# hadleyhzy34/porl

Measured on AMD Instinct MI355X. Metric: gradient-steps/sec (POR update, batch=1024), higher is better.
Workload: dtype f32; 1 GPU; POR S=60 A=2 H=1024 L=2 B=1024/GPU (global 1024), 1000000 -row replay (1000000/GPU) resident in HBM, device sampler + gather + full update per step; parallelism=dp1, global_batch=1024

## Files before the change

### include/porl_hip.h

```cpp
#ifndef PORL_HIP_H
#define PORL_HIP_H

#include <stdint.h>

#ifdef __cplusplus
extern "C" {
#endif

#define PORL_ABI_VERSION 11
#define PORL_MAX_HIDDEN 8

#define PORL_OK 0
#define PORL_ERR_INVALID (-1)
#define PORL_ERR_UNSUPPORTED (-2)
#define PORL_ERR_UNBOUND (-3)

int porl_abi_version(void);
const char* porl_last_error(void);

typedef struct porl_iql_cfg {
  int32_t obs_dim;
  int32_t pol_out_dim;
  int32_t hidden_dim;
  int32_t n_hidden;
  int32_t layer_norm;
  int32_t pol_tanh;
  int32_t weight_mode;
  int32_t max_batch;
} porl_iql_cfg;

typedef struct porl_iql porl_iql;

int porl_iql_create(const porl_iql_cfg* cfg, porl_iql** out);
void porl_iql_destroy(porl_iql* h);

int64_t porl_iql_group_floats(const porl_iql* h, int group);
int32_t porl_iql_group_tensors(const porl_iql* h, int group);
int porl_iql_tensor_info(const porl_iql* h, int group, int index, int64_t* offset, int32_t* rows,
                         int32_t* cols);

int64_t porl_iql_workspace_floats(const porl_iql* h);

typedef struct porl_iql_buffers {
  float* params_vf;
  float* params_tgt;
  float* params_pol;
  float* grads_vf;
  float* grads_pol;
  float* adam_m_vf;
  float* adam_v_vf;
  float* adam_m_pol;
  float* adam_v_pol;
  float* workspace;
  float* stats;
} porl_iql_buffers;

int porl_iql_bind(porl_iql* h, const porl_iql_buffers* bufs);

int porl_iql_load_batch(porl_iql* h, int32_t batch,
                        const float* obs, int64_t obs_rs,
                        const float* next_obs, int64_t next_rs,
                        const float* rew, int64_t rew_rs,
                        const float* term, int64_t term_rs,
                        const float* pol_target, int64_t pt_rs,
// ... 428 lines not shown
```

### porl_amd/_native.py

```python
from __future__ import annotations

import ctypes as C
import os

_HERE = os.path.dirname(os.path.abspath(__file__))
LIB_PATH = os.path.join(_HERE, "lib", "libporl_hip.so")

ABI_VERSION = 11

SYMBOLS = [
    "porl_abi_version", "porl_last_error",
    "porl_iql_create", "porl_iql_destroy", "porl_iql_group_floats", "porl_iql_group_tensors",
    "porl_iql_tensor_info", "porl_iql_workspace_floats", "porl_iql_bind", "porl_iql_load_batch",
    "porl_iql_load_batch_sampled", "porl_iql_load_batch_indexed", "porl_iql_set_stats", "porl_iql_set_mode", "porl_iql_tune_set",
    "porl_iql_value_backward", "porl_iql_value_apply", "porl_iql_policy_forward", "porl_iql_policy_backward",
    "porl_iql_policy_apply", "porl_iql_step", "porl_iql_policy_only_forward", "porl_iql_policy_only_step", "porl_iql_policy_prefetch", "porl_iql_forward_value", "porl_iql_forward_policy",
    "porl_gemm_f32", "porl_gemm_f32_group", "porl_adam_ema", "porl_ema", "porl_softmax_mask", "porl_gather_rows", "porl_sample_indices", "porl_epoch_indices", "porl_per_update", "porl_per_sample",
    "porl_per_record", "porl_per_sample_slots", "porl_per_update_f32",
    "porl_prof_enable", "porl_prof_read", "porl_tune_set", "porl_tune_set_ptr", "porl_state2costmap", "porl_astar_label",
    "porl_signal_create", "porl_signal_destroy", "porl_signal_write", "porl_signal_wait_ge", "porl_iql_update_pipelined",
    "porl_qnet_create", "porl_qnet_destroy", "porl_qnet_param_floats", "porl_qnet_tensors",
    "porl_qnet_tensor_info", "porl_qnet_workspace_floats", "porl_qnet_bind", "porl_qnet_load_batch",
    "porl_qnet_cql_backward", "porl_qnet_apply", "porl_qnet_learn", "porl_qnet_sync_target",
    "porl_qnet_forward", "porl_qnet_forward_loaded", "porl_qnet_backward", "porl_qr_loss", "porl_iqn_quantile_huber", "porl_iqn_cos_embed", "porl_iqn_hadamard", "porl_iqn_hadamard_backward", "porl_iqn_select", "porl_iqn_scatter", "porl_iqn_target", "porl_grad_clip", "porl_c51_loss", "porl_reduce_mean", "porl_qnet_penalty", "porl_qnet_learn_indexed", "porl_qnet_one_launch", "porl_qnet_learn_variant", "porl_qnet_can_sample", "porl_qnet_learn_sampled", "porl_qnet_dist_learn",
    "porl_qnet_record", "porl_qnet_act_ok", "porl_qnet_act",
    "porl_qnet_learn_sampled_variant", "porl_qnet_bcq_mask", "porl_qnet_bcq_learn", "porl_qnet_bcq_learn_sampled",
    "porl_iqn_create", "porl_iqn_destroy", "porl_iqn_workspace_floats", "porl_iqn_bind", "porl_iqn_learn", "porl_iqn_act",
    "porl_iqn_mix", "porl_iqn_head",
    "porl_enc_create", "porl_enc_destroy", "porl_enc_param_floats", "porl_enc_stat_floats",
    "porl_enc_workspace_floats", "porl_enc_tensors", "porl_enc_norms", "porl_enc_blocks",
    "porl_enc_tensor_info", "porl_enc_norm_info", "porl_enc_bind", "porl_enc_weights_changed", "porl_enc_forward", "porl_enc_forward_rows",
    "porl_enc_tap_info",
    "porl_episode_workspace", "porl_episode_count", "porl_episode_fill", "porl_episode_returns", "porl_hindsight_pairs",
    "porl_gather_pairs",
]

# ... 97 lines not shown


class NativeError(RuntimeError):
    pass


_lib = None


def _declare(lib):
    vp, i32, i64, f32, f64 = C.c_void_p, C.c_int32, C.c_int64, C.c_float, C.c_double
    lib.porl_abi_version.restype = C.c_int
    lib.porl_last_error.restype = C.c_char_p
    lib.porl_iql_create.argtypes = [C.POINTER(IqlCfg), C.POINTER(vp)]
    lib.porl_iql_destroy.argtypes = [vp]
    lib.porl_iql_destroy.restype = None
    lib.porl_iql_group_floats.argtypes = [vp, C.c_int]
    lib.porl_iql_group_floats.restype = i64
    lib.porl_iql_group_tensors.argtypes = [vp, C.c_int]
    lib.porl_iql_group_tensors.restype = i32
    lib.porl_iql_tensor_info.argtypes = [vp, C.c_int, C.c_int, C.POINTER(i64), C.POINTER(i32), C.POINTER(i32)]
    lib.porl_iql_workspace_floats.argtypes = [vp]
    lib.porl_iql_workspace_floats.restype = i64
    lib.porl_iql_bind.argtypes = [vp, C.POINTER(IqlBuffers)]
    lib.porl_iql_load_batch.argtypes = [vp, i32, vp, i64, vp, i64, vp, i64, vp, i64, vp, i64, vp]
    lib.porl_iql_load_batch_sampled.argtypes = [vp, i32, vp, i64, i64, i32, i32, C.c_uint64, C.c_uint64, vp, vp]
    lib.porl_iql_load_batch_indexed.argtypes = [vp, i32, vp, i64, i64, vp, i32, i32, i32, i32, vp, i64, vp, i64, vp]
    lib.porl_iql_set_stats.argtypes = [vp, vp]
    lib.porl_iql_set_mode.argtypes = [vp, i32]
    for name in ("porl_iql_value_backward", "porl_iql_value_apply", "porl_iql_policy_forward", "porl_iql_policy_backward",
                 "porl_iql_policy_apply", "porl_iql_step", "porl_iql_policy_only_forward", "porl_iql_policy_only_step"):
        getattr(lib, name).argtypes = [vp, C.POINTER(IqlHyper), vp]
    lib.porl_iql_policy_prefetch.argtypes = [vp, vp]
    lib.porl_iql_forward_value.argtypes = [vp, C.c_int, vp, i64, i32, vp, vp, vp]
    lib.porl_iql_forward_policy.argtypes = [vp, vp, i64, i32, vp, i64, vp]
    lib.porl_gemm_f32.argtypes = [C.c_int, C.c_int, i32, i32, i32, vp, i32, vp, i32, vp, i32, vp, C.c_int,
                                  vp, i32, C.c_int, vp, vp]
    lib.porl_gemm_f32_group.argtypes = [C.POINTER(GemmDesc), i32, C.c_int, C.c_int, vp]
    lib.porl_adam_ema.argtypes = [vp, vp, vp, vp, vp, i64, f64, i32, f64, f64, f64, f64, vp]
    lib.porl_ema.argtypes = [vp, vp, i64, f64, vp]
    lib.porl_softmax_mask.argtypes = [vp, i64, i32, i32, f32, i32, vp, vp]
    lib.porl_gather_rows.argtypes = [vp, i64, vp, i32, i32, vp, i64, vp]
    lib.porl_sample_indices.argtypes = [i64, i32, C.c_uint64, C.c_uint64, i64, vp, vp]
    lib.porl_epoch_indices.argtypes = [i64, i64, i32, C.c_uint64, C.c_uint64, i64, vp, vp]
    lib.porl_per_update.argtypes = [vp, i64, vp, vp, i32, f64, f64, vp, vp]
    lib.porl_per_sample.argtypes = [vp, i64, vp, i32, i64, f64, vp, vp, vp, vp]
# ... 141 lines not shown
```

### porl_amd/csrc/gemm_f32.hpp

```cpp
#pragma once
#include <hip/hip_runtime.h>
#include <stdint.h>

#ifndef PORL_ABL
#define PORL_ABL 0
#endif

namespace porl {

enum : int { ACT_NONE = 0, ACT_RELU = 1, ACT_TANH = 2 };

enum : int {
  APRO_NONE = 0,
  APRO_AFFINE_RELU = 1,
};

struct GemmProb {
  const float* A;
  const float* B;
  float* C;
  const float* bias;
  const float* mask;
  const float* headw;
  float* headout;
  float* colsum;
  const float* a_colscale;
  const float* a_colshift;
  const float* resid;
  const float* rscale;
  float* cstat;
  int rs_rows, rs_row0;
  int a_grp, a_grp_jump, a_seg_tiles, a_seg_jump;
  int M, N, K;
  int lda, ldb, ldc, ldmask;
  int act;
  int apro;
  int splitk;
  int store_c;
  int a_vec, b_vec;
  int a_kc, b_kc;
  int c_vec;
  int tiles_m, tiles_n, block_start, kchunk;
};

constexpr int MAX_GROUP = 8;
struct GemmGroup {
  int nprob;
  int total_blocks;
  int single_buffer;
  GemmProb p[MAX_GROUP];
  int lds_pad, lds_pad_min_blocks;
};

// ... 20 lines not shown
  const unsigned long long a = reinterpret_cast<unsigned long long>(p);
  BufRsrc r;
  r.x = (int)(unsigned)(a & 0xFFFFFFFFull);
  r.y = (int)(unsigned)((a >> 32) & 0xFFFFull);
  r.z = (int)(bytes >= 0x7FFFFFFFull ? 0x7FFFFFFFu : (unsigned)bytes);
  r.w = 0x00020000;
  return r;
}
__device__ __forceinline__ float4 buf_ld128(BufRsrc r, unsigned voff, unsigned soff) {
  const f32x4 v = llvm_raw_buffer_load_v4f32(r, (int)voff, (int)soff, 0);
  return make_float4(v.x, v.y, v.z, v.w);
}
__device__ __forceinline__ float buf_ld32(BufRsrc r, unsigned voff, unsigned soff) {
  return llvm_raw_buffer_load_f32(r, (int)voff, (int)soff, 0);
}

template <bool V> struct BoolTag { static constexpr bool value = V; };
template <int V> struct IntTag { static constexpr int value = V; };

#ifdef PORL_STAMP
__device__ unsigned long long g_stamps[16 * 4096];
#endif

template <int BM, int BN, int BK, int WM, int WN, bool VEC, bool APRO, bool ONEBUF = false>
__global__ __launch_bounds__(64 * WM * WN) void gemm_f32_kernel(const GemmGroup g) {
  constexpr int THREADS = 64 * WM * WN;
  constexpr int WTM = BM / WM / 32;
  constexpr int WTN = BN / WN / 32;
  constexpr int SA = lds_stride(BM);
  constexpr int SB = lds_stride(BN);
  constexpr int SK = BK + 4;
  constexpr int A_TILE = (BK * SA > BM * SK) ? BK * SA : BM * SK;
  constexpr int B_TILE = (BK * SB > BN * SK) ? BK * SB : BN * SK;
  static_assert(BK % 8 == 0, "a k-group is 8 wide");
  constexpr int NLA = BM * BK / 4 / THREADS;
  constexpr int NLB = BN * BK / 4 / THREADS;
  static_assert(NLA >= 1 && NLB >= 1, "tile too small for the thread count");
  static_assert(BM * BK / 4 % THREADS == 0 && BN * BK / 4 % THREADS == 0, "staging must divide evenly");
  static_assert(BK % 4 == 0 && WTM >= 1 && WTN >= 1 && BM % (32 * WM) == 0 && BN % (32 * WN) == 0, "tile shape");

  constexpr int APRO_MAX_K = ONEBUF ? 512 : 1024;
  constexpr int NBUF = ONEBUF ? 1 : 2;
  __shared__ __attribute__((aligned(16))) float lds[NBUF * (A_TILE + B_TILE) + (APRO ? 2 * APRO_MAX_K : 0)];

  const int t = threadIdx.x;
  const int lane = t & 63;
  const int wave = t >> 6;
// ... 379 lines not shown

  auto run = [&](auto guard_tag) {
    if (a_kc && b_kc) {
      main_loop(guard_tag, BoolTag<true>{}, BoolTag<true>{}, BoolTag<false>{});
    } else if constexpr (APRO) {
    } else if (a_kc) {
      main_loop(guard_tag, BoolTag<true>{}, BoolTag<false>{}, BoolTag<false>{});
    } else if (do_colsum) {
      main_loop(guard_tag, BoolTag<false>{}, BoolTag<false>{}, BoolTag<true>{});
    } else {
      main_loop(guard_tag, BoolTag<false>{}, BoolTag<false>{}, BoolTag<false>{});
    }
  };
  if constexpr (VEC) {
    if (full) run(BoolTag<false>{});
    else run(BoolTag<true>{});
  } else {
    run(BoolTag<true>{});
  }
#ifdef PORL_STAMP
  if (t == 0) { rt_loop1 = __builtin_amdgcn_s_memrealtime(); cy1 = __builtin_amdgcn_s_memtime(); }
#endif

  if (do_colsum) {
    __syncthreads();
    float4* red = reinterpret_cast<float4*>(lds);
    constexpr int C4 = BM / 4;
    auto reduce_cols = [&](const float4& mine, float* out) {
      red[t] = mine;
      __syncthreads();
      if (t < C4) {
        float4 s = red[t];
        for (int u = t + C4; u < THREADS; u += C4) {
          const float4 o = red[u];
          s.x += o.x; s.y += o.y; s.z += o.z; s.w += o.w;
        }
        const int c = m0 + t * 4;
        if (c < M) out[c] = s.x;
        if (c + 1 < M) out[c + 1] = s.y;
        if (c + 2 < M) out[c + 2] = s.z;
        if (c + 3 < M) out[c + 3] = s.w;
      }
      __syncthreads();
    };
    reduce_cols(csum, P.colsum + (size_t)split * M);
  }

  const bool raw = P.splitk > 1;
  float* __restrict__ Cg = P.C + (raw ? (size_t)split * M * P.ldc : 0);
  const bool has_head = (!raw) && P.headw != nullptr;
  const float* __restrict__ maskp = raw ? nullptr : P.mask;
  const int act = raw ? ACT_NONE : P.act;
  const bool store_c = P.store_c != 0;
  constexpr int WROWS = BM / WM, WCOLS = BN / WN, CS = WCOLS + 4;
  static_assert(WM * WN * WROWS * CS <= NBUF * (A_TILE + B_TILE), "C sub-tiles must fit in the staging LDS");
  const bool fast_c = store_c && P.c_vec && (m0 + BM <= M) && (n0 + BN <= N);
  float* ctile = lds + wave * (WROWS * CS);
#pragma unroll
  for (int i = 0; i < WTM; ++i) {
    const int rbase = m0 + wm * (BM / WM) + i * 32 + 4 * kh;
#pragma unroll
    for (int j = 0; j < WTN; ++j) {
      const int col = n0 + wn * (BN / WN) + j * 32 + li;
      const bool col_ok = col < N;
      float bv = 0.f, hw = 0.f;
      if (!raw && col_ok) {
        if (P.bias) bv = P.bias[col];
        if (has_head) hw = P.headw[col];
      }
      float vals[16];
#pragma unroll
      for (int r = 0; r < 16; ++r) {
        float v = acc[i][j][r] + bv;
        if (act == ACT_RELU) v = fmaxf(v, 0.f);
        else if (act == ACT_TANH) v = tanhf(v);
        vals[r] = v;
      }
      if (maskp && !fast_c) {
#pragma unroll
        for (int r = 0; r < 16; ++r) {
// ... 25 lines not shown
        cs += __shfl_xor(cs, 32);
        cq += __shfl_xor(cq, 32);
        const int rblk = (m0 + wm * (BM / WM)) / 32 + i;
        if (kh == 0 && col_ok && rblk * 32 < M) {
          float* o = P.cstat + (size_t)rblk * 2 * N + col;
          o[0] = cs;
          o[N] = cq;
        }
      }
      if (has_head) {
        const int part = (n0 + wn * (BN / WN) + j * 32) >> 5;
#pragma unroll
        for (int r = 0; r < 16; ++r) {
          float sh = vals[r] * hw;
          sh += __shfl_xor(sh, 16);
          sh += __shfl_xor(sh, 8);
          sh += __shfl_xor(sh, 4);
          sh += __shfl_xor(sh, 2);
          sh += __shfl_xor(sh, 1);
          const int row = rbase + (r & 3) + 8 * (r >> 2);
          if (li == 0 && row < M && part * 32 < N) P.headout[(size_t)part * M + row] = sh;
        }
      }
      if (store_c) {
        if (fast_c) {
#pragma unroll
          for (int r = 0; r < 16; ++r)
            ctile[(i * 32 + (r & 3) + 8 * (r >> 2) + 4 * kh) * CS + j * 32 + li] = vals[r];
        } else {
#pragma unroll
          for (int r = 0; r < 16; ++r) {
            const int row = rbase + (r & 3) + 8 * (r >> 2);
            if (row < M && col_ok) Cg[(size_t)row * P.ldc + col] = vals[r];
          }
        }
      }
    }
  }
  if (fast_c) {
    constexpr int C4 = WCOLS / 4;
    const int wr0 = m0 + wm * WROWS, wc0 = n0 + wn * WCOLS;
#pragma unroll 4
    for (int f = lane; f < WROWS * C4; f += 64) {
      const int r = f / C4, c = (f % C4) * 4;
      float4 v = *reinterpret_cast<const float4*>(ctile + r * CS + c);
      if (maskp) {
        const float4 mk = *reinterpret_cast<const float4*>(maskp + (size_t)(wr0 + r) * P.ldmask + wc0 + c);
        v.x = mk.x > 0.f ? v.x : 0.f; v.y = mk.y > 0.f ? v.y : 0.f;
        v.z = mk.z > 0.f ? v.z : 0.f; v.w = mk.w > 0.f ? v.w : 0.f;
      }
      if (!raw && P.resid) {
        const float rs = P.rscale ? P.rscale[(wr0 + r + P.rs_row0) / P.rs_rows] : 1.f;
        const float4 x4 = *reinterpret_cast<const float4*>(P.resid + (size_t)(wr0 + r) * P.ldc + wc0 + c);
        v.x = __fadd_rn(x4.x, __fmul_rn(v.x, rs)); v.y = __fadd_rn(x4.y, __fmul_rn(v.y, rs));
        v.z = __fadd_rn(x4.z, __fmul_rn(v.z, rs)); v.w = __fadd_rn(x4.w, __fmul_rn(v.w, rs));
      }
      *reinterpret_cast<float4*>(Cg + (size_t)(wr0 + r) * P.ldc + wc0 + c) = v;
    }
// ... 65 lines not shown
    if (p.splitk < 1) p.splitk = 1;
    int kc = (p.K + p.splitk - 1) / p.splitk;
    kc = ((kc + GEMM_BK - 1) / GEMM_BK) * GEMM_BK;
    p.kchunk = kc;
    p.c_vec = aligned16(p.C) && (p.ldc % 4 == 0) && (p.splitk == 1 || ((size_t)p.M * p.ldc) % 4 == 0) &&
              (p.mask == nullptr || (aligned16(p.mask) && p.ldmask % 4 == 0));
    p.block_start = start;
    start += p.tiles_m * p.tiles_n * p.splitk;
  }
  g.total_blocks = start;
  return start;
}

template <int BM, int BN, int WM, int WN>
inline hipError_t launch_tile(const GemmGroup& g, hipStream_t s) {
  dim3 grid(g.total_blocks), block(64 * WM * WN);
  const int pad = g.total_blocks >= g.lds_pad_min_blocks ? g.lds_pad : 0;
  bool vec = true, apro = g.p[0].apro != APRO_NONE;
  for (int i = 0; i < g.nprob; ++i) {
    vec = vec && g.p[i].a_vec && g.p[i].b_vec;
    if ((g.p[i].apro != APRO_NONE) != apro) return hipErrorInvalidValue;
    if (g.p[i].splitk <= 1 && (g.p[i].mask || g.p[i].resid) && (g.p[i].cstat || g.p[i].headw)) return hipErrorInvalidValue;
  }
  if (apro) {
    if constexpr ((BM == 64 && BN == 64) || (BM == 128 && BN == 64) || (BM == 128 && BN == 96)) {
      for (int i = 0; i < g.nprob; ++i) {
        const GemmProb& p = g.p[i];
        if (!p.a_kc || !p.b_kc || p.K % GEMM_BK || p.splitk > 1 || !p.a_colscale || !p.a_colshift || !vec ||
            (reinterpret_cast<uintptr_t>(p.a_colscale) & 15u) || (reinterpret_cast<uintptr_t>(p.a_colshift) & 15u))
          return hipErrorInvalidValue;
        if (p.K > (g.single_buffer && BM == 64 && BN == 64 ? 512 : 1024)) return hipErrorInvalidValue;
      }
      if constexpr (BM == 64 && BN == 64) {
        if (g.single_buffer) {
          hipLaunchKernelGGL((gemm_f32_kernel<BM, BN, GEMM_BK, WM, WN, true, true, true>), grid, block, pad, s, g);
          return hipGetLastError();
        }
      }
      hipLaunchKernelGGL((gemm_f32_kernel<BM, BN, GEMM_BK, WM, WN, true, true>), grid, block, pad, s, g);
      return hipGetLastError();
    } else {
      return hipErrorInvalidValue;
    }
  }
  if constexpr (BM == 64 && BN == 64) {
    if (vec && g.single_buffer) {
// ... 38 lines not shown
```

### porl_amd/csrc/porl_api.hip

```cpp
#include <hip/hip_runtime.h>

#include <algorithm>
#include <cmath>
#include <cstdio>
#include <cstring>
#include <string>
#include <vector>

#include "../../include/porl_hip.h"
#include "gemm_f32.hpp"
#include "gemm_bf16.hpp"
#include "kernels.hpp"
#include "l0_fwd.hpp"
#include "skinny.hpp"
#include "iqn.hpp"
#include "qnet_fused.hpp"
#include "per_tree.hpp"
#include "dist_losses.hpp"
#include "online.hpp"
#include "per_online.hpp"
#include "bcq_mask.hpp"
#include "astar.hpp"
#include "episodes.hpp"

// ... 85 lines not shown
    (void)hipEventRecord(r.e1, s);
    g_prof.recs.push_back(r);
  }
};

const float* g_dbg_a_scale = nullptr; const float* g_dbg_a_shift = nullptr; const float* g_dbg_resid = nullptr;
float* g_dbg_cstat = nullptr;
unsigned long long* g_qnet_stamps = nullptr;

constexpr int NUM_CU = 256;
constexpr int SK_MAX = 16;
constexpr int NLL_ROWS_PER_BLOCK = 4;
constexpr int LN_ROWS_PER_BLOCK = 8;
constexpr int HEAD_ROWS_PER_BLOCK = HEAD_ROWS;

struct Tune {
  int tile_map[4] = {TILE_64x128, TILE_64x64, TILE_64x128, TILE_64x64};
  int tile_map_short[4] = {TILE_64x64, TILE_64x64, TILE_64x128, TILE_64x64};
  int vbwd_tile_short = -1;
  int l0_kernel = 1;
  int l0_tile = -1;
  int skinny = 7;
  int skinny_pipelined = -1, skinny_pipelined_max_h = 768;
  int dw0_slabs = 16;
  int iql_fold = 1;
  int gemm_lds_pad = 0, gemm_lds_pad_min_blocks = 0;
  int iql_pad_value = 18432, iql_pad_policy = 0, iql_pad_min_blocks = 4 * NUM_CU, iql_pad_min_k = 0;
  int enc_tile_n96 = 0;
  int enc_gemm_sb = 1;
  int enc_patch_rows = 0;
  int enc_s2d = 0;
  int enc_bf16_operands_only = 0;
  int enc_pconv_mfma = 0;
  int enc_bn_sweep = 0;
  int enc_dense_patch = 0;
  int qnet_fused = 1;
  int qnet_rows16 = 1;
  int qnet_wgrad_share = 11;
  int qnet_two_groups = 1;
} g_tune;

enum TuneClamp { TC_ANY, TC_BOOL, TC_NONNEG, TC_1_16, TC_MASK };
struct TuneKey { const char* key; int Tune::*field; TuneClamp clamp; };
#define TK(key, clamp) {#key, &Tune::key, clamp}
const TuneKey k_tune_keys[] = {
    TK(gemm_lds_pad, TC_NONNEG), TK(gemm_lds_pad_min_blocks, TC_NONNEG), TK(iql_pad_value, TC_NONNEG), TK(iql_pad_policy, TC_NONNEG),
    TK(iql_pad_min_blocks, TC_NONNEG), TK(iql_pad_min_k, TC_NONNEG), TK(qnet_fused, TC_BOOL), TK(qnet_two_groups, TC_BOOL),
    TK(qnet_wgrad_share, TC_1_16), TK(qnet_rows16, TC_BOOL), TK(enc_dense_patch, TC_BOOL), TK(enc_s2d, TC_BOOL), TK(enc_patch_rows, TC_NONNEG),
    TK(enc_gemm_sb, TC_ANY), TK(enc_tile_n96, TC_BOOL), TK(enc_bn_sweep, TC_BOOL), TK(enc_pconv_mfma, TC_BOOL), TK(enc_bf16_operands_only, TC_BOOL),
    TK(iql_fold, TC_BOOL), TK(skinny, TC_MASK), TK(skinny_pipelined, TC_MASK), TK(skinny_pipelined_max_h, TC_ANY), TK(dw0_slabs, TC_1_16),
    TK(l0_tile, TC_ANY), TK(l0_kernel, TC_BOOL), TK(vbwd_tile_short, TC_ANY),
};

int tune_apply(Tune& t, const char* key, int value) {
  if (!key) PORL_FAIL(PORL_ERR_INVALID, "null key");
  for (const TuneKey& k : k_tune_keys) {
    if (strcmp(key, k.key)) continue;
    const TuneClamp c = k.clamp;
    t.*k.field = c == TC_BOOL ? value != 0 : c == TC_NONNEG ? std::max(0, value) : c == TC_1_16 ? std::max(1, std::min(value, 16))
               : c == TC_MASK && value == 1 ? 7 : value;
    return PORL_OK;
  }
  const bool sh = !strncmp(key, "tile_map_short", 14);
  const char* i = key + (sh ? 14 : 8);
  if (!strncmp(key, "tile_map", 8) && *i >= '0' && *i <= '3' && !i[1] && value >= 0 && value < TILE_COUNT) {
    (sh ? t.tile_map_short : t.tile_map)[*i - '0'] = value;
    return PORL_OK;
  }
  PORL_FAIL(PORL_ERR_INVALID, "unknown tuning key '%s'", key);
}

inline int64_t ru4(int64_t x) { return (x + 3) & ~int64_t(3); }
inline int cdiv(int a, int b) { return (a + b - 1) / b; }
// ... 91 lines not shown
  else if (minN <= 64) { cand[nc++] = TILE_128x64; cand[nc++] = TILE_64x64; }
  else if (minM <= 64) { cand[nc++] = TILE_64x128; cand[nc++] = TILE_64x64; }
  else { cand[nc++] = TILE_128x128; cand[nc++] = TILE_128x64; cand[nc++] = TILE_64x64; }
  const int* map = short_blocks ? t.tile_map_short : t.tile_map;
  for (int i = 0; i < nc; ++i)
    if (blocks(cand[i]) >= NUM_CU) return map[cand[i]];
  return map[cand[nc - 1]];
}

int pick_splitk(int M, int N, int K, int nprob, int bm, int bn) {
  const int tiles = nprob * cdiv(M, bm) * cdiv(N, bn);
  int sk = cdiv(NUM_CU, tiles);
  sk = std::min(sk, std::max(1, K / 64));
  return std::max(1, std::min(sk, SK_MAX));
}

int launch_group(GemmGroup& g, int tile, const Tune& t, hipStream_t s, int iql_pad = -1) {
  const bool iql = iql_pad >= 0 && !t.gemm_lds_pad && g.nprob > 0 && g.p[0].K >= t.iql_pad_min_k;
  g.lds_pad = iql ? iql_pad : t.gemm_lds_pad;
  g.lds_pad_min_blocks = iql ? t.iql_pad_min_blocks : t.gemm_lds_pad_min_blocks;
  double flops = 0.0, bytes = 0.0;
  std::string label;
  if (g_prof.on) {
    bool vec = true, apro = false;
    for (int i = 0; i < g.nprob; ++i) {
      const GemmProb& p = g.p[i];
      flops += 2.0 * p.M * p.N * p.K;
      bytes += 4.0 * ((double)p.M * p.K + (double)p.N * p.K + (p.store_c ? (double)p.M * p.N : 0.0));
      vec = vec && p.a_vec && p.b_vec;
      apro = apro || p.apro != APRO_NONE;
    }
    int bm, bn;
    tile_dims(tile, bm, bn);
    const TileCfg tc = tile_cfg(tile);
    label = "gemm_f32_kernel<" + std::to_string(bm) + "," + std::to_string(bn) + "," + std::to_string(GEMM_BK) + "," +
            std::to_string(tc.wm) + "," + std::to_string(tc.wn) + "," + (vec ? "true" : "false") + "," +
            (apro ? "true" : "false") + (g.single_buffer && vec && tile == TILE_64x64 ? ",true>" : ">");
  }
  ProfScope ps(label, s, flops, bytes);
  hipError_t e = launch_gemm_group(tile, g, s);
  if (e != hipSuccess) {
    g_err = std::string("gemm launch: ") + hipGetErrorString(e);
    return (int)e;
  }
  return 0;
}

int launch_group_bf16(GemmGroup& g, int tile, hipStream_t s) {
  double flops = 0.0, bytes = 0.0;
  std::string label;
  if (g_prof.on) {
    for (int i = 0; i < g.nprob; ++i) {
      const GemmProb& p = g.p[i];
      flops += 2.0 * p.M * p.N * p.K;
      bytes += 4.0 * ((double)p.M * p.K + (double)p.N * p.K + (double)p.M * p.N * (p.resid ? 2.0 : 1.0));
    }
    int bm, bn;
    tile_dims(tile, bm, bn);
    label = "gemm_bf16_kernel<" + std::to_string(bm) + "," + std::to_string(bn) + "," +
            (g.p[0].apro != APRO_NONE ? "true" : "false") + ">";
// ... 175 lines not shown
  }
  w.pol_w = take(B);
  w.total = o;
  *out = h;
  return PORL_OK;
}

void porl_iql_destroy(porl_iql* h) { delete h; }

int64_t porl_iql_group_floats(const porl_iql* h, int group) { return !h ? 0 : (group == 0 ? h->n_vf : h->n_pol); }
int32_t porl_iql_group_tensors(const porl_iql* h, int group) {
  return !h ? 0 : (int32_t)(group == 0 ? h->t_vf.size() : h->t_pol.size());
}
int porl_iql_tensor_info(const porl_iql* h, int group, int index, int64_t* offset, int32_t* rows, int32_t* cols) {
  if (!h || group < 0 || group > 1) PORL_FAIL(PORL_ERR_INVALID, "bad group");
  const auto& v = group == 0 ? h->t_vf : h->t_pol;
  if (index < 0 || index >= (int)v.size()) PORL_FAIL(PORL_ERR_INVALID, "tensor index out of range");
  if (offset) *offset = v[index].off;
  if (rows) *rows = v[index].rows;
  if (cols) *cols = v[index].cols;
  return PORL_OK;
}
int64_t porl_iql_workspace_floats(const porl_iql* h) { return h ? h->ws.total : 0; }

int porl_iql_bind(porl_iql* h, const porl_iql_buffers* b) {
  if (!h || !b) PORL_FAIL(PORL_ERR_INVALID, "null argument");
  const void* ptrs[] = {b->params_vf, b->params_tgt, b->params_pol, b->grads_vf, b->grads_pol, b->adam_m_vf,
                        b->adam_v_vf, b->adam_m_pol, b->adam_v_pol, b->workspace, b->stats};
  for (const void* p : ptrs) {
    if (!p) PORL_FAIL(PORL_ERR_INVALID, "null buffer");
    if (!aligned16(p)) PORL_FAIL(PORL_ERR_INVALID, "buffers must be 16-byte aligned");
  }
  h->buf = *b;
  h->bound = true;
  h->device = device_of(b->workspace);
  h->batch = 0;
  return PORL_OK;
}

int porl_iql_load_batch(porl_iql* h, int32_t batch, const float* obs, int64_t obs_rs, const float* next_obs,
                        int64_t next_rs, const float* rew, int64_t rew_rs, const float* term, int64_t term_rs,
                        const float* pol_target, int64_t pt_rs, void* stream) {
  PORL_TRY(check_ready(h, false)); DevGuard _dg(h->device);
  if (batch < 1 || batch > h->cfg.max_batch) PORL_FAIL(PORL_ERR_INVALID, "batch %d outside [1,%d]", batch, h->cfg.max_batch);
  if (!obs || !next_obs || !rew || !term) PORL_FAIL(PORL_ERR_INVALID, "null batch tensor");
  float* W = h->buf.workspace;
// ... 196 lines not shown
  for (int i = 0; i < nnets; ++i) if (!skn_ok4(nets[i].dz, ldz)) return false;
  WgradSkinnyArgs a{};
  a.nnets = nnets; a.B = B; a.H = H; a.S = S; a.ldz = ldz; a.ldx = ldx; a.ldo = S;
  a.tiles_n = cdiv(H, SKN_T);
  skn_split(cdiv(B, SKN_T), h->tune.dw0_slabs, a.nslab, a.rtiles);
  a.slabW_stride = (long)H * S; a.slabC_stride = H;
  for (int i = 0; i < nnets; ++i) {
    a.net[i] = WgradSkinnyNet{nets[i].dz, X, nets[i].slabW, nets[i].slabC};
    add_reduce(red, nets[i].gw, nets[i].slabW, (long)H * S, (long)H * S, a.nslab);
    add_reduce(red, nets[i].gb, nets[i].slabC, H, H, a.nslab);
  }
  g_phase = phase;
  {
    ProfScope ps("wgrad_skinny_kernel", s, 2.0 * nnets * B * (double)H * S,
                 4.0 * nnets * ((double)B * H + (double)B * S + (double)a.nslab * H * (S + 1)));
    hipLaunchKernelGGL(wgrad_skinny_kernel, dim3(nnets * a.nslab * a.tiles_n), dim3(256), 0, s, a);
  }
  g_phase = "";
  const hipError_t e = hipGetLastError();
  if (e != hipSuccess) { g_err = std::string("wgrad_skinny_kernel: ") + hipGetErrorString(e); *rc = (int)e; }
  return true;
}

static int value_backward_impl(porl_iql* h, const porl_iql_hyper* hp, hipStream_t s, ReduceArgs* defer) {
  const int B = h->batch, S = h->cfg.obs_dim, H = h->cfg.hidden_dim, L = h->cfg.n_hidden, Hp = h->Hp;
  float* W = h->buf.workspace;
  const Workspace& ws = h->ws;
  const float* Pv = h->buf.params_vf;
  const float* Pt = h->buf.params_tgt;
  float* Gv = h->buf.grads_vf;
  int parts = 0;
  const bool LN = h->cfg.layer_norm != 0;

  for (int l = 0; l < L; ++l) {
    FwdNet nets[4];
    const int K = l == 0 ? S : H;
    for (int n = 0; n < 4; ++n) {
      const bool tgt = n < 2;
      const int i = n & 1;
      const float* P = tgt ? Pt : Pv;
      FwdNet& f = nets[n];
      if (l == 0) { f.in = W + (tgt ? ws.xn : ws.xs_slot[h->slot]); f.ldin = h->Sp; }
      else { f.in = W + (tgt ? ws.act_t[i][(l - 1) & 1] : ws.act_v[i][l - 1]); f.ldin = Hp; }
      f.W = P + h->v[i].w[l]; f.b = P + h->v[i].b[l];
      const bool last = l == L - 1;
      f.out = tgt ? ((last && !LN) ? nullptr : W + ws.act_t[i][l & 1]) : W + ws.act_v[i][l];
// ... 25 lines not shown

  ReduceArgs red{};
  if (LN) return value_backward_ln(h, hp, s, defer);
  {
    const int nhb = cdiv(B, HEAD_ROWS_PER_BLOCK);
    HeadBwdArgs a{};
    for (int i = 0; i < 2; ++i) {
      a.Hact[i] = W + ws.act_v[i][L - 1]; a.w[i] = Pv + h->v[i].w[L];
      a.dZ[i] = W + ws.dz_v[i][(L - 1) & 1]; a.part_dw[i] = W + ws.head_part[i];
      a.hp_t[i] = W + ws.hp_t[i]; a.hp_v[i] = W + ws.hp_v[i];
      a.b_t[i] = Pt + h->v[i].b[L]; a.b_v[i] = Pv + h->v[i].b[L];
      a.dv[i] = W + ws.dv[i]; a.part_db[i] = W + ws.head_db[i];
      add_reduce(red, Gv + h->v[i].w[L], W + ws.head_part[i], H, H, nhb);
      add_reduce(red, Gv + h->v[i].b[L], W + ws.head_db[i], 1, 1, nhb);
    }
    a.rew = W + ws.rew; a.term = W + ws.term; a.target_v = W + ws.target_v_slot[h->slot]; a.part_loss = W + ws.head_loss;
    add_reduce(red, h->buf.stats, W + ws.head_loss, 1, 1, nhb, 0, hp->inv_batch);
    a.B = B; a.H = H; a.ld = Hp; a.parts = parts;
    a.tau = hp->tau; a.discount = hp->discount; a.inv_batch = hp->inv_batch;
    ProfScope ps("relu_head_bwd_kernel", s, 0.0, 16.0 * B * H);
    hipLaunchKernelGGL(relu_head_bwd_kernel, dim3(nhb, 2), dim3(256), 0, s, a);
    PORL_HIP(hipGetLastError());
  }
  for (int l = L - 1; l >= 0; --l) {
    const int Kin = l == 0 ? S : H;
    if (l == 0) {
      Dw0Net dn[2];
      const int64_t per = (int64_t)H * S, perc = H;
      for (int i = 0; i < 2; ++i) {
        float* slabW = W + ws.slab_a + (int64_t)i * SK_MAX * (per + 2 * perc + 8);
        dn[i] = Dw0Net{W + ws.dz_v[i][0], Gv + h->v[i].w[0], Gv + h->v[i].b[0], slabW, slabW + (int64_t)SK_MAX * per};
      }
      int rc = 0;
      if (dw0_skinny(h, dn, 2, W + ws.xs_slot[h->slot], h->Sp, B, H, S, Hp, red, "V6.dW0:", s, &rc)) {
        if (rc) return rc;
        break;
      }
    }
    GemmGroup g{};
    for (int i = 0; i < 2; ++i) {
      const float* dz = W + ws.dz_v[i][l & 1];
      const float* in = l == 0 ? W + ws.xs_slot[h->slot] : W + ws.act_v[i][l - 1];
      const int ldin = l == 0 ? h->Sp : Hp;
      GemmProb p = make_prob(GEMM_TN, dz, Hp, in, ldin, Gv + h->v[i].w[l], Kin, H, Kin, B);
      p.colsum = Gv + h->v[i].b[l];
      g.p[g.nprob++] = p;
      if (l > 0) {
        GemmProb q = make_prob(GEMM_NN, dz, Hp, Pv + h->v[i].w[l], Kin, W + ws.dz_v[i][(l - 1) & 1], Hp, B, Kin, H);
        q.mask = W + ws.act_v[i][l - 1]; q.ldmask = Hp;
        g.p[g.nprob++] = q;
      }
    }
    int tile = iql_tile(h, g);
    if (l > 0 && short_blocks(h) && h->tune.vbwd_tile_short >= 0) tile = h->tune.vbwd_tile_short;
    if (l == 0) {
      int bm, bn;
      tile_dims(tile, bm, bn);
      const int sk = pick_splitk(H, Kin, B, 2, bm, bn);
      if (sk > 1) {
        const int64_t per = (int64_t)H * Kin, perc = H;
        for (int i = 0; i < 2; ++i) {
          float* slabW = W + ws.slab_a + (int64_t)i * SK_MAX * (per + 2 * perc + 8);
          float* slabC = slabW + (int64_t)SK_MAX * per;
          g.p[i].splitk = sk; g.p[i].C = slabW; g.p[i].colsum = slabC;
          add_reduce(red, Gv + h->v[i].w[0], slabW, per, per, sk);
          add_reduce(red, Gv + h->v[i].b[0], slabC, perc, perc, sk);
        }
      }
    }
    g_phase = l == 0 ? "V6.dW0:" : "V5.bwd:";
    PORL_TRY(iql_launch(h, g, tile, false, s));
  }
  g_phase = "V7.combine:";
  if (defer) *defer = red;
  else PORL_TRY(launch_reduce(red, s));
  g_phase = "";
  return PORL_OK;
// ... 271 lines not shown
    g_phase = "";
    PORL_HIP(hipGetLastError());
  } else {
    GemmGroup g{};
    g.nprob = 2;
    g.p[0] = make_prob(GEMM_TN, W + ws.dmu, Dp, W + ws.act_p[L - 1], Hp, Gp + h->pol.w[L], H, D, H, B);
    g.p[0].colsum = Gp + h->pol.b[L];
    g.p[1] = make_prob(GEMM_NN, W + ws.dmu, Dp, Pp + h->pol.w[L], H, W + ws.dz_p[(L - 1) & 1], Hp, B, H, D);
    g.p[1].mask = W + ws.act_p[L - 1]; g.p[1].ldmask = Hp;
    const int tile = D <= 64 ? TILE_64x128 : iql_tile(h, g);
    int bm, bn;
    tile_dims(tile, bm, bn);
    const int sk = pick_splitk(D, H, B, 1, bm, bn);
    if (sk > 1) {
      float* slabW = W + ws.slab_b;
      float* slabC = slabW + (int64_t)SK_MAX * D * H;
      g.p[0].splitk = sk; g.p[0].C = slabW; g.p[0].colsum = slabC;
      add_reduce(red, Gp + h->pol.w[L], slabW, (long)D * H, (long)D * H, sk);
      add_reduce(red, Gp + h->pol.b[L], slabC, D, D, sk);
    }
    g_phase = "P5.outbwd:";
    PORL_TRY(iql_launch(h, g, tile, true, s));
  }
  for (int l = L - 1; l >= 0; --l) {
    const int Kin = l == 0 ? S : H;
    if (l == 0) {
      const int64_t per = (int64_t)H * S;
      float* slabW = W + ws.slab_pa;
      Dw0Net dn{W + ws.dz_p[0], Gp + h->pol.w[0], Gp + h->pol.b[0], slabW, slabW + (int64_t)SK_MAX * per};
      int rc = 0;
      if (dw0_skinny(h, &dn, 1, W + ws.xs_slot[h->slot], h->Sp, B, H, S, Hp, red, "P7.dW0:", s, &rc)) {
        if (rc) return rc;
        break;
      }
    }
    const float* dz = W + ws.dz_p[l & 1];
    const float* in = l == 0 ? W + ws.xs_slot[h->slot] : W + ws.act_p[l - 1];
    const int ldin = l == 0 ? h->Sp : Hp;
    GemmGroup g{};
    g.p[g.nprob] = make_prob(GEMM_TN, dz, Hp, in, ldin, Gp + h->pol.w[l], Kin, H, Kin, B);
    g.p[g.nprob++].colsum = Gp + h->pol.b[l];
    if (l > 0) {
      GemmProb q = make_prob(GEMM_NN, dz, Hp, Pp + h->pol.w[l], Kin, W + ws.dz_p[(l - 1) & 1], Hp, B, Kin, H);
      q.mask = W + ws.act_p[l - 1]; q.ldmask = Hp;
      g.p[g.nprob++] = q;
    }
    const int tile = iql_tile(h, g);
    if (l == 0) {
      int bm, bn;
      tile_dims(tile, bm, bn);
      const int sk = pick_splitk(H, Kin, B, 1, bm, bn);
      if (sk > 1) {
        const int64_t per = (int64_t)H * Kin;
        float* slabW = W + ws.slab_pa;
        float* slabC = slabW + (int64_t)SK_MAX * per;
        g.p[0].splitk = sk; g.p[0].C = slabW; g.p[0].colsum = slabC;
        add_reduce(red, Gp + h->pol.w[0], slabW, per, per, sk);
        add_reduce(red, Gp + h->pol.b[0], slabC, H, H, sk);
      }
    }
    g_phase = l == 0 ? "P7.dW0:" : "P6.bwd:";
    PORL_TRY(iql_launch(h, g, tile, true, s));
  }
  g_phase = "P8.combine:";
  if (defer) *defer = red;
  else PORL_TRY(launch_reduce(red, s));
  g_phase = "";
  return PORL_OK;
}

// ... 634 lines not shown
```

### porl_amd/engine.py

```python
from __future__ import annotations

import ctypes as C
import math

import numpy as np
import torch

from . import _native as N


def _norm_device(device):
    device = torch.device(device)
    if device.type == "cuda" and device.index is None:
        device = torch.device("cuda", torch.cuda.current_device())
    return device


class IqlEngine:
    GROUP_VF, GROUP_POL = 0, 1
    MODE_TWO_SLOTS, MODE_FOLD_COMBINE, MODE_SHORT_BLOCKS = 1, 2, 4
    SLOTS = 3

    def __init__(self, obs_dim, pol_out_dim, hidden_dim, n_hidden, layer_norm=False, pol_tanh=False,
                 weight_mode=0, max_batch=1024, device="cpu"):
# ... 118 lines not shown
            self._free_signals()
        self._side, self._events = None, []
        self._policy_done = self._values_read = None
        for name in ("params_vf", "params_tgt", "params_pol", "grads_vf", "grads_pol", "adam_m_vf",
                     "adam_v_vf", "adam_m_pol", "adam_v_pol", "stats"):
            setattr(self, name, getattr(self, name).to(device))
        self.device = device
        self.workspace = None
        self._bound = False
        return self

    def tensor_table(self, group):
        n = int(self._lib.porl_iql_group_tensors(self._h, group))
        out = []
        off, r, c = C.c_int64(), C.c_int32(), C.c_int32()
        for i in range(n):
            N.check(self._lib.porl_iql_tensor_info(self._h, group, i, C.byref(off), C.byref(r), C.byref(c)))
            out.append((off.value, (c.value,) if r.value == 0 else (r.value, c.value)))
        return out

    @staticmethod
    def views(flat, table):
        return [flat[o:o + math.prod(shape)].view(shape) for o, shape in table]

    @staticmethod
    def _mat(t, cols, what):
        if t.dtype != torch.float32:
            raise RuntimeError(f"{what}: expected float32, got {t.dtype}")
        if t.dim() != 2 or t.shape[1] != cols:
            raise RuntimeError(f"{what}: expected shape (B, {cols}), got {tuple(t.shape)}")
        if t.stride(1) != 1:
            t = t.contiguous()
        return t

    def _vec(self, t, B, what):
        if t.dim() != 1 or t.shape[0] != B:
            raise RuntimeError(f"{what}: expected shape ({B},), got {tuple(t.shape)}")
        return t if t.dtype == torch.float32 else t.float()

    def load_batch(self, obs, next_obs, rew, term, pol_target=None):
        self._ensure_bound()
        for t in (obs, next_obs, rew, term, pol_target):
            if t is not None and t.device != self.device:
                raise RuntimeError(f"batch tensor on {t.device}, engine on {self.device}")
        S, D = self.cfg.obs_dim, self.cfg.pol_out_dim
        obs, next_obs = self._mat(obs, S, "observations"), self._mat(next_obs, S, "next_observations")
# ... 323 lines not shown
```

Baseline: 3122 gradient-steps/sec.

## Fuse first-layer weight gradient into layer-1 backward GEMM epilogue

Adds a DW0 "rider" mode to the f32 GEMM kernel. While the layer-1 backward NN GEMM produces dz0 tiles, the epilogue multiplies them against the input observation slab with MFMA and writes per-64-row partial dW0 and bias-gradient slabs, which are later reduced. Layer 0 no longer needs its own dW0 launch and dz0 no longer has to be written and re-read, for both value nets and the policy net. In exchange the tile is forced to BM=64, register and LDS pressure grows in the epilogue, and more partial slabs must be reduced. It also adds a workspace-offset query for inspecting intermediate matrices.

```diff
diff --git a/include/porl_hip.h b/include/porl_hip.h
--- a/include/porl_hip.h
+++ b/include/porl_hip.h
@@ -40,6 +40,7 @@
                          int32_t* cols);
 
 int64_t porl_iql_workspace_floats(const porl_iql* h);
+int64_t porl_iql_workspace_offset(const porl_iql* h, const char* what, int net, int layer);
 
 typedef struct porl_iql_buffers {
   float* params_vf;
diff --git a/porl_amd/_native.py b/porl_amd/_native.py
--- a/porl_amd/_native.py
+++ b/porl_amd/_native.py
@@ -11,7 +11,7 @@
 SYMBOLS = [
     "porl_abi_version", "porl_last_error",
     "porl_iql_create", "porl_iql_destroy", "porl_iql_group_floats", "porl_iql_group_tensors",
-    "porl_iql_tensor_info", "porl_iql_workspace_floats", "porl_iql_bind", "porl_iql_load_batch",
+    "porl_iql_tensor_info", "porl_iql_workspace_floats", "porl_iql_workspace_offset", "porl_iql_bind", "porl_iql_load_batch",
     "porl_iql_load_batch_sampled", "porl_iql_load_batch_indexed", "porl_iql_set_stats", "porl_iql_set_mode", "porl_iql_tune_set",
     "porl_iql_value_backward", "porl_iql_value_apply", "porl_iql_policy_forward", "porl_iql_policy_backward",
     "porl_iql_policy_apply", "porl_iql_step", "porl_iql_policy_only_forward", "porl_iql_policy_only_step", "porl_iql_policy_prefetch", "porl_iql_forward_value", "porl_iql_forward_policy",
@@ -155,6 +155,8 @@
     lib.porl_iql_tensor_info.argtypes = [vp, C.c_int, C.c_int, C.POINTER(i64), C.POINTER(i32), C.POINTER(i32)]
     lib.porl_iql_workspace_floats.argtypes = [vp]
     lib.porl_iql_workspace_floats.restype = i64
+    lib.porl_iql_workspace_offset.argtypes = [vp, C.c_char_p, C.c_int, C.c_int]
+    lib.porl_iql_workspace_offset.restype = i64
     lib.porl_iql_bind.argtypes = [vp, C.POINTER(IqlBuffers)]
     lib.porl_iql_load_batch.argtypes = [vp, i32, vp, i64, vp, i64, vp, i64, vp, i64, vp, i64, vp]
     lib.porl_iql_load_batch_sampled.argtypes = [vp, i32, vp, i64, i64, i32, i32, C.c_uint64, C.c_uint64, vp, vp]
diff --git a/porl_amd/csrc/gemm_f32.hpp b/porl_amd/csrc/gemm_f32.hpp
--- a/porl_amd/csrc/gemm_f32.hpp
+++ b/porl_amd/csrc/gemm_f32.hpp
@@ -29,6 +29,11 @@
   const float* resid;
   const float* rscale;
   float* cstat;
+  const float* dw0_x;
+  float* dw0_w;
+  float* dw0_b;
+  long dw0_wstride;
+  int dw0_ldx, dw0_s;
   int rs_rows, rs_row0;
   int a_grp, a_grp_jump, a_seg_tiles, a_seg_jump;
   int M, N, K;
@@ -95,7 +100,7 @@
 __device__ unsigned long long g_stamps[16 * 4096];
 #endif
 
-template <int BM, int BN, int BK, int WM, int WN, bool VEC, bool APRO, bool ONEBUF = false>
+template <int BM, int BN, int BK, int WM, int WN, bool VEC, bool APRO, bool ONEBUF = false, bool DW0 = false>
 __global__ __launch_bounds__(64 * WM * WN) void gemm_f32_kernel(const GemmGroup g) {
   constexpr int THREADS = 64 * WM * WN;
   constexpr int WTM = BM / WM / 32;
@@ -521,6 +526,23 @@
   if (t == 0) { rt_loop1 = __builtin_amdgcn_s_memrealtime(); cy1 = __builtin_amdgcn_s_memtime(); }
 #endif
 
+  [[maybe_unused]] float xf[2][16];
+  [[maybe_unused]] bool rider = false;
+  if constexpr (DW0) {
+    static_assert(BM == 64 && WM == 2 && WTM == 1 && VEC && !APRO && !ONEBUF, "the rider's slabs are 64 rows = two waves of 32");
+    rider = P.dw0_x != nullptr;
+    if (rider) {
+      const int xr0 = m0 + wm * 32 + 4 * kh;
+#pragma unroll
+      for (int jb = 0; jb < 2; ++jb)
+#pragma unroll
+        for (int r = 0; r < 16; ++r) {
+          const int row = xr0 + (r & 3) + 8 * (r >> 2), xc = jb * 32 + li;
+          xf[jb][r] = (row < M && xc < P.dw0_s) ? P.dw0_x[(size_t)row * P.dw0_ldx + xc] : 0.f;
+        }
+    }
+  }
+
   if (do_colsum) {
     __syncthreads();
     float4* red = reinterpret_cast<float4*>(lds);
@@ -555,6 +577,10 @@
   static_assert(WM * WN * WROWS * CS <= NBUF * (A_TILE + B_TILE), "C sub-tiles must fit in the staging LDS");
   const bool fast_c = store_c && P.c_vec && (m0 + BM <= M) && (n0 + BN <= N);
   float* ctile = lds + wave * (WROWS * CS);
+  constexpr int XT = 16 * 64 + 32, XW = WTN * XT;
+  static_assert(!DW0 || WM * WN * XW <= NBUF * (A_TILE + B_TILE), "the rider's exchange must fit in the staging LDS");
+  [[maybe_unused]] f32x16 dkeep[WTN];
+  [[maybe_unused]] float cskeep[WTN];
 #pragma unroll
   for (int i = 0; i < WTM; ++i) {
     const int rbase = m0 + wm * (BM / WM) + i * 32 + 4 * kh;
@@ -626,6 +652,31 @@
           if (li == 0 && row < M && part * 32 < N) P.headout[(size_t)part * M + row] = sh;
         }
       }
+      if constexpr (DW0) {
+        if (rider) {
+          f32x16 d0, d1;
+#pragma unroll
+          for (int r = 0; r < 16; ++r) { d0[r] = 0.f; d1[r] = 0.f; }
+#pragma unroll
+          for (int r = 0; r < 16; ++r) d0 = __builtin_amdgcn_mfma_f32_32x32x2f32(vals[r], xf[0][r], d0, 0, 0, 0);
+          if (P.dw0_s > 32) {
+#pragma unroll
+            for (int r = 0; r < 16; ++r) d1 = __builtin_amdgcn_mfma_f32_32x32x2f32(vals[r], xf[1][r], d1, 0, 0, 0);
+          }
+          float cs = 0.f;
+#pragma unroll
+          for (int r = 0; r < 16; ++r) cs += vals[r];
+          cs += __shfl_xor(cs, 32);
+          float* xw = lds + wave * XW + j * XT;
+#pragma unroll
+          for (int r = 0; r < 16; ++r) {
+            xw[r * 64 + lane] = wm ? d0[r] : d1[r];
+            dkeep[j][r] = wm ? d1[r] : d0[r];
+          }
+          if (kh == 0) xw[16 * 64 + li] = cs;
+          cskeep[j] = cs;
+        }
+      }
       if (store_c) {
         if (fast_c) {
 #pragma unroll
@@ -638,6 +689,30 @@
             if (row < M && col_ok) Cg[(size_t)row * P.ldc + col] = vals[r];
           }
         }
+      }
+    }
+  }
+  if constexpr (DW0) {
+    if (rider) {
+      __syncthreads();
+      const int S = P.dw0_s;
+      float* __restrict__ ow = P.dw0_w + (size_t)tm * P.dw0_wstride;
+      const float* pw = lds + ((1 - wm) * WN + wn) * XW;
+      const int xc = wm * 32 + li;
+#pragma unroll
+      for (int j = 0; j < WTN; ++j) {
+        const int c0 = n0 + wn * (BN / WN) + j * 32;
+        if (xc < S) {
+#pragma unroll
+          for (int r = 0; r < 16; ++r) {
+            const int c = c0 + (r & 3) + 8 * (r >> 2) + 4 * kh;
+            const float other = pw[j * XT + r * 64 + lane];
+            const float v = wm ? other + dkeep[j][r] : dkeep[j][r] + other;
+            if (c < N) ow[(size_t)c * S + xc] = v;
+          }
+        }
+        if (wm == 0 && kh == 0 && c0 + li < N)
+          P.dw0_b[(size_t)tm * N + c0 + li] = cskeep[j] + pw[j * XT + 16 * 64 + li];
       }
     }
   }
@@ -749,6 +824,24 @@
     if ((g.p[i].apro != APRO_NONE) != apro) return hipErrorInvalidValue;
     if (g.p[i].splitk <= 1 && (g.p[i].mask || g.p[i].resid) && (g.p[i].cstat || g.p[i].headw)) return hipErrorInvalidValue;
   }
+  bool dw0 = false;
+  for (int i = 0; i < g.nprob; ++i) {
+    const GemmProb& p = g.p[i];
+    if (!p.dw0_x) continue;
+    if (p.splitk > 1 || p.store_c || p.resid || p.cstat || p.headw || !p.dw0_w || !p.dw0_b || p.dw0_s < 1 || p.dw0_s > 64 ||
+        p.dw0_ldx < p.dw0_s || p.dw0_wstride < (long)p.N * p.dw0_s)
+      return hipErrorInvalidValue;
+    dw0 = true;
+  }
+  if (dw0) {
+    if constexpr (BM == 64 && (BN == 64 || BN == 128)) {
+      if (!vec || apro || g.single_buffer) return hipErrorInvalidValue;
+      hipLaunchKernelGGL((gemm_f32_kernel<BM, BN, GEMM_BK, WM, WN, true, false, false, true>), grid, block, pad, s, g);
+      return hipGetLastError();
+    } else {
+      return hipErrorInvalidValue;
+    }
+  }
   if (apro) {
     if constexpr ((BM == 64 && BN == 64) || (BM == 128 && BN == 64) || (BM == 128 && BN == 96)) {
       for (int i = 0; i < g.nprob; ++i) {
diff --git a/porl_amd/csrc/porl_api.hip b/porl_amd/csrc/porl_api.hip
--- a/porl_amd/csrc/porl_api.hip
+++ b/porl_amd/csrc/porl_api.hip
@@ -131,6 +131,7 @@
   int l0_tile = -1;
   int skinny = 7;
   int skinny_pipelined = -1, skinny_pipelined_max_h = 768;
+  int dw0_epilogue = 1;
   int dw0_slabs = 16;
   int iql_fold = 1;
   int gemm_lds_pad = 0, gemm_lds_pad_min_blocks = 0;
@@ -157,7 +158,7 @@
     TK(iql_pad_min_blocks, TC_NONNEG), TK(iql_pad_min_k, TC_NONNEG), TK(qnet_fused, TC_BOOL), TK(qnet_two_groups, TC_BOOL),
     TK(qnet_wgrad_share, TC_1_16), TK(qnet_rows16, TC_BOOL), TK(enc_dense_patch, TC_BOOL), TK(enc_s2d, TC_BOOL), TK(enc_patch_rows, TC_NONNEG),
     TK(enc_gemm_sb, TC_ANY), TK(enc_tile_n96, TC_BOOL), TK(enc_bn_sweep, TC_BOOL), TK(enc_pconv_mfma, TC_BOOL), TK(enc_bf16_operands_only, TC_BOOL),
-    TK(iql_fold, TC_BOOL), TK(skinny, TC_MASK), TK(skinny_pipelined, TC_MASK), TK(skinny_pipelined_max_h, TC_ANY), TK(dw0_slabs, TC_1_16),
+    TK(iql_fold, TC_BOOL), TK(skinny, TC_MASK), TK(skinny_pipelined, TC_MASK), TK(skinny_pipelined_max_h, TC_ANY), TK(dw0_slabs, TC_1_16), TK(dw0_epilogue, TC_BOOL),
     TK(l0_tile, TC_ANY), TK(l0_kernel, TC_BOOL), TK(vbwd_tile_short, TC_ANY),
 };
 
@@ -295,11 +296,16 @@
   double flops = 0.0, bytes = 0.0;
   std::string label;
   if (g_prof.on) {
-    bool vec = true, apro = false;
+    bool vec = true, apro = false, dw0 = false;
     for (int i = 0; i < g.nprob; ++i) {
       const GemmProb& p = g.p[i];
       flops += 2.0 * p.M * p.N * p.K;
       bytes += 4.0 * ((double)p.M * p.K + (double)p.N * p.K + (p.store_c ? (double)p.M * p.N : 0.0));
+      if (p.dw0_x) {
+        dw0 = true;
+        flops += 2.0 * p.M * p.N * p.dw0_s;
+        bytes += 4.0 * ((double)p.M * p.dw0_s + (double)cdiv(p.M, 64) * p.N * (p.dw0_s + 1));
+      }
       vec = vec && p.a_vec && p.b_vec;
       apro = apro || p.apro != APRO_NONE;
     }
@@ -308,7 +314,7 @@
     const TileCfg tc = tile_cfg(tile);
     label = "gemm_f32_kernel<" + std::to_string(bm) + "," + std::to_string(bn) + "," + std::to_string(GEMM_BK) + "," +
             std::to_string(tc.wm) + "," + std::to_string(tc.wn) + "," + (vec ? "true" : "false") + "," +
-            (apro ? "true" : "false") + (g.single_buffer && vec && tile == TILE_64x64 ? ",true>" : ">");
+            (apro ? "true" : "false") + (dw0 ? ",false,true>" : g.single_buffer && vec && tile == TILE_64x64 ? ",true>" : ">");
   }
   ProfScope ps(label, s, flops, bytes);
   hipError_t e = launch_gemm_group(tile, g, s);
@@ -530,6 +536,16 @@
   return PORL_OK;
 }
 int64_t porl_iql_workspace_floats(const porl_iql* h) { return h ? h->ws.total : 0; }
+int64_t porl_iql_workspace_offset(const porl_iql* h, const char* what, int net, int layer) {
+  if (!h || !what || net < 0 || net > 1 || layer < 0 || layer >= h->cfg.n_hidden) return -1;
+  const Workspace& w = h->ws;
+  if (!strcmp(what, "xs")) return w.xs_slot[h->slot];
+  if (!strcmp(what, "act_v")) return w.act_v[net][layer];
+  if (!strcmp(what, "dz_v")) return w.dz_v[net][layer & 1];
+  if (!strcmp(what, "act_p")) return w.act_p[layer];
+  if (!strcmp(what, "dz_p")) return w.dz_p[layer & 1];
+  return -1;
+}
 
 int porl_iql_bind(porl_iql* h, const porl_iql_buffers* b) {
   if (!h || !b) PORL_FAIL(PORL_ERR_INVALID, "null argument");
@@ -772,6 +788,35 @@
   return true;
 }
 
+static bool dw0_rider(const porl_iql* h, GemmGroup& g, int& tile, const Dw0Net* nets, int nnets, const float* X, int ldx,
+                      int B, int H, int S, ReduceArgs& red) {
+  const int nslab = cdiv(B, 64);
+  if (!h->tune.dw0_epilogue || h->cfg.n_hidden < 2 || h->cfg.layer_norm || S > 64 || nslab > SK_MAX || !skn_ok4(X, ldx)) return false;
+  for (int i = 0; i < g.nprob; ++i) if (!g.p[i].a_vec || !g.p[i].b_vec) return false;
+  GemmProb nn[MAX_GROUP], rest[MAX_GROUP];
+  int n_nn = 0, n_rest = 0;
+  for (int i = 0; i < g.nprob; ++i) {
+    if (g.p[i].a_kc && !g.p[i].b_kc) nn[n_nn++] = g.p[i];
+    else rest[n_rest++] = g.p[i];
+  }
+  if (n_nn != nnets) return false;
+  for (int i = 0; i < nnets; ++i) {
+    GemmProb& p = nn[i];
+    p.dw0_x = X; p.dw0_ldx = ldx; p.dw0_s = S;
+    p.dw0_w = nets[i].slabW; p.dw0_wstride = (long)H * S; p.dw0_b = nets[i].slabC;
+    p.store_c = 0;
+    add_reduce(red, nets[i].gw, nets[i].slabW, (long)H * S, (long)H * S, nslab);
+    add_reduce(red, nets[i].gb, nets[i].slabC, H, H, nslab);
+  }
+  g.nprob = 0;
+  for (int i = 0; i < n_nn; ++i) g.p[g.nprob++] = nn[i];
+  for (int i = 0; i < n_rest; ++i) g.p[g.nprob++] = rest[i];
+  int bm, bn;
+  tile_dims(tile, bm, bn);
+  if (bm != 64) tile = bn >= 128 ? TILE_64x128 : TILE_64x64;
+  return true;
+}
+
 static int value_backward_impl(porl_iql* h, const porl_iql_hyper* hp, hipStream_t s, ReduceArgs* defer) {
   const int B = h->batch, S = h->cfg.obs_dim, H = h->cfg.hidden_dim, L = h->cfg.n_hidden, Hp = h->Hp;
   float* W = h->buf.workspace;
@@ -843,15 +888,16 @@
     hipLaunchKernelGGL(relu_head_bwd_kernel, dim3(nhb, 2), dim3(256), 0, s, a);
     PORL_HIP(hipGetLastError());
   }
-  for (int l = L - 1; l >= 0; --l) {
+  Dw0Net dn[2];
+  for (int i = 0; i < 2; ++i) {
+    const int64_t per = (int64_t)H * S, perc = H;
+    float* slabW = W + ws.slab_a + (int64_t)i * SK_MAX * (per + 2 * perc + 8);
+    dn[i] = Dw0Net{W + ws.dz_v[i][0], Gv + h->v[i].w[0], Gv + h->v[i].b[0], slabW, slabW + (int64_t)SK_MAX * per};
+  }
+  bool dw0_done = false;
+  for (int l = L - 1; l >= 0 && !dw0_done; --l) {
     const int Kin = l == 0 ? S : H;
     if (l == 0) {
-      Dw0Net dn[2];
-      const int64_t per = (int64_t)H * S, perc = H;
-      for (int i = 0; i < 2; ++i) {
-        float* slabW = W + ws.slab_a + (int64_t)i * SK_MAX * (per + 2 * perc + 8);
-        dn[i] = Dw0Net{W + ws.dz_v[i][0], Gv + h->v[i].w[0], Gv + h->v[i].b[0], slabW, slabW + (int64_t)SK_MAX * per};
-      }
       int rc = 0;
       if (dw0_skinny(h, dn, 2, W + ws.xs_slot[h->slot], h->Sp, B, H, S, Hp, red, "V6.dW0:", s, &rc)) {
         if (rc) return rc;
@@ -874,6 +920,7 @@
     }
     int tile = iql_tile(h, g);
     if (l > 0 && short_blocks(h) && h->tune.vbwd_tile_short >= 0) tile = h->tune.vbwd_tile_short;
+    if (l == 1) dw0_done = dw0_rider(h, g, tile, dn, 2, W + ws.xs_slot[h->slot], h->Sp, B, H, S, red);
     if (l == 0) {
       int bm, bn;
       tile_dims(tile, bm, bn);
@@ -1191,12 +1238,11 @@
     g_phase = "P5.outbwd:";
     PORL_TRY(iql_launch(h, g, tile, true, s));
   }
-  for (int l = L - 1; l >= 0; --l) {
+  const Dw0Net dn{W + ws.dz_p[0], Gp + h->pol.w[0], Gp + h->pol.b[0], W + ws.slab_pa, W + ws.slab_pa + (int64_t)SK_MAX * H * S};
+  bool dw0_done = false;
+  for (int l = L - 1; l >= 0 && !dw0_done; --l) {
     const int Kin = l == 0 ? S : H;
     if (l == 0) {
-      const int64_t per = (int64_t)H * S;
-      float* slabW = W + ws.slab_pa;
-      Dw0Net dn{W + ws.dz_p[0], Gp + h->pol.w[0], Gp + h->pol.b[0], slabW, slabW + (int64_t)SK_MAX * per};
       int rc = 0;
       if (dw0_skinny(h, &dn, 1, W + ws.xs_slot[h->slot], h->Sp, B, H, S, Hp, red, "P7.dW0:", s, &rc)) {
         if (rc) return rc;
@@ -1214,7 +1260,8 @@
       q.mask = W + ws.act_p[l - 1]; q.ldmask = Hp;
       g.p[g.nprob++] = q;
     }
-    const int tile = iql_tile(h, g);
+    int tile = iql_tile(h, g);
+    if (l == 1) dw0_done = dw0_rider(h, g, tile, &dn, 1, W + ws.xs_slot[h->slot], h->Sp, B, H, S, red);
     if (l == 0) {
       int bm, bn;
       tile_dims(tile, bm, bn);
diff --git a/porl_amd/engine.py b/porl_amd/engine.py
--- a/porl_amd/engine.py
+++ b/porl_amd/engine.py
@@ -164,6 +164,14 @@
     @staticmethod
     def views(flat, table):
         return [flat[o:o + math.prod(shape)].view(shape) for o, shape in table]
+
+    def workspace_matrix(self, what, rows, net=0, layer=0):
+        off = int(self._lib.porl_iql_workspace_offset(self._h, what.encode(), net, layer))
+        if off < 0:
+            raise N.NativeError(f"no workspace matrix {what!r} for net {net}, layer {layer}")
+        cols = self.cfg.obs_dim if what == "xs" else self.cfg.hidden_dim
+        ld = (cols + 3) // 4 * 4
+        return self.workspace[off:off + rows * ld].view(rows, ld)[:, :cols]
 
     @staticmethod
     def _mat(t, cols, what):
```

Result: slower. 3056 gradient-steps/sec (-2.1%).
